# lashhw/rtcuda

Hardware: AMD Instinct MI355X
Metric: Msamples/s at 1920x1080, bun_zipper.ply (higher is better)
Workload: dtype f32

## Files before the change

### rtcuda_amd/csrc/rt_device.h

```cpp
#ifndef RT_DEVICE_H
#define RT_DEVICE_H

#include <hip/hip_runtime.h>
#include <stdint.h>

#include "rt_pinned_math.h"

#define RT_DEV __device__ __forceinline__
#ifdef RT_ISA_MARKS
#define RT_MARK(name) __asm__ volatile("; RT_MARK " name)
#else
#define RT_MARK(name)
#endif

namespace rt {

constexpr float kInvPi = 0.31830988618379067153f;
constexpr float kTwoPi = 6.28318530717958647692f;
constexpr int kRrStart = 4;
constexpr float kRrThreshold = 1.f;
constexpr float kFltMax = 3.402823466e+38f;
constexpr float kFltEps = 1.192092896e-07f;

struct V3 {
    float x, y, z;
};
RT_DEV V3 mk(float x, float y, float z) { return V3{x, y, z}; }
RT_DEV V3 neg(V3 a) { return mk(-a.x, -a.y, -a.z); }
RT_DEV V3 add(V3 a, V3 b) { return mk(a.x + b.x, a.y + b.y, a.z + b.z); }
RT_DEV V3 sub(V3 a, V3 b) { return mk(a.x - b.x, a.y - b.y, a.z - b.z); }
RT_DEV V3 mul(V3 a, V3 b) { return mk(a.x * b.x, a.y * b.y, a.z * b.z); }
RT_DEV V3 scale(V3 a, float t) { return mk(a.x * t, a.y * t, a.z * t); }
RT_DEV V3 divf(V3 a, float t) {
    float inv_t = 1.f / t;
    return mk(a.x * inv_t, a.y * inv_t, a.z * inv_t);
}
RT_DEV float dot(V3 a, V3 b) { return a.x * b.x + a.y * b.y + a.z * b.z; }
RT_DEV V3 cross(V3 a, V3 b) {
    return mk(a.y * b.z - a.z * b.y, a.z * b.x - a.x * b.z, a.x * b.y - a.y * b.x);
}
RT_DEV float len2(V3 a) { return a.x * a.x + a.y * a.y + a.z * a.z; }
RT_DEV float len(V3 a) { return sqrtf(a.x * a.x + a.y * a.y + a.z * a.z); }
RT_DEV V3 unit(V3 a) {
    float inv_len = 1.f / len(a);
    return mk(a.x * inv_len, a.y * inv_len, a.z * inv_len);
}
RT_DEV float max3(V3 a) { return fmaxf(fmaxf(a.x, a.y), a.z); }
template <int STEPS = 1>
RT_DEV float rcp_exact_normal(float x) {
    float r = __builtin_amdgcn_rcpf(x);
#pragma unroll
    for (int k = 0; k < STEPS; k++) {
        const float e = fmaf(-x, r, 1.f);
        r = fmaf(e, r, r);
    }
    return r;
}
RT_DEV V3 reflect(V3 v, V3 n) { return sub(v, scale(n, 2.f * dot(v, n))); }
RT_DEV V3 refract4(V3 unit_v, V3 unit_n, float eta_ratio, float cos_theta) {
    V3 v_parallel = scale(add(unit_v, scale(unit_n, cos_theta)), eta_ratio);
    V3 v_perp = scale(unit_n, -sqrtf(1.f - len2(v_parallel)));
    return add(v_parallel, v_perp);
}

struct Rng {
    uint32_t d, v0, v1, v2, v3, v4;
};
constexpr uint32_t kRngWeyl = 362437u;
RT_DEV void rng_step(Rng &s) {
    uint32_t t = s.v0 ^ (s.v0 >> 2);
    s.v0 = s.v1;
    s.v1 = s.v2;
    s.v2 = s.v3;
    s.v3 = s.v4;
    s.v4 = (s.v4 ^ (s.v4 << 4)) ^ (t ^ (t << 1));
}
RT_DEV uint32_t rng_next(Rng &s) {
    rng_step(s);
    s.d += kRngWeyl;
    return s.v4 + s.d;
}
RT_DEV Rng rng_sample_stream(uint32_t seed_lo, uint32_t seed_hi, unsigned long long key) {
    unsigned long long z = (((unsigned long long)seed_hi << 32) | seed_lo) + 0x9E3779B97F4A7C15ull * (key + 1ull);
    z = (z ^ (z >> 30)) * 0xBF58476D1CE4E5B9ull;
    z = (z ^ (z >> 27)) * 0x94D049BB133111EBull;
    z ^= z >> 31;
    const uint32_t s0 = (uint32_t)z ^ 0xaad26b49u, s1 = (uint32_t)(z >> 32) ^ 0xf7dcefddu;
    const uint32_t t0 = 1099087573u * s0, t1 = 2591861531u * s1;
    Rng r;
    r.d = 6615241u + t1 + t0;
    r.v0 = 123456789u + t0;
    r.v1 = 362436069u ^ t0;
    r.v2 = 521288629u + t1;
    r.v3 = 88675123u ^ t1;
    r.v4 = 5783321u + t0;
    return r;
}
RT_DEV float rng_to_uniform(uint32_t draw) { return (float)draw * 2.3283064e-10f + (2.3283064e-10f / 2.0f); }
RT_DEV float rng_uniform(Rng &s) { return rng_to_uniform(rng_next(s)); }

struct Tri {
    V3 p0, e1, e2, n;
};
RT_DEV Tri load_tri(const float4 *__restrict__ tris, int k) {
    const float4 *q = (const float4 *)((const char *)tris + __umul24((unsigned)k, 48u));
    float4 a = q[0];
    float4 b = q[1];
    float4 c = q[2];
    Tri t;
    t.p0 = mk(a.x, a.y, a.z);
    t.e1 = mk(a.w, b.x, b.y);
    t.e2 = mk(b.z, b.w, c.x);
    t.n = mk(c.y, c.z, c.w);
    return t;
}
RT_DEV bool tri_intersect(const Tri &tr, V3 o, V3 d, float tmax, float &t_out, float &u_out, float &v_out) {
    V3 c = sub(tr.p0, o);
    V3 r = cross(d, c);
    float inv_det = 1.f / dot(d, tr.n);
    float u = inv_det * dot(tr.e2, r);
    float v = inv_det * dot(tr.e1, r);
    float t = inv_det * dot(c, tr.n);
    t_out = t;
    u_out = u;
    v_out = v;
    return u >= 0.0f && v >= 0.0f && (u + v) <= 1.0f && 0 < t && t <= tmax;
}
RT_DEV V3 tri_point(const Tri &tr, float u, float v) { return add(sub(tr.p0, scale(tr.e1, u)), scale(tr.e2, v)); }
RT_DEV float tri_area(const Tri &tr) { return 0.5f * len(tr.n); }

RT_DEV V3 offset_ray_origin(V3 p, V3 n) {
    const float int_scale = 256.f;
    const float float_scale = 1.f / 65536.f;
    const float origin = 1.f / 32.f;
    int ox = (int)(int_scale * n.x);
    int oy = (int)(int_scale * n.y);
    int oz = (int)(int_scale * n.z);
    float px = __int_as_float(__float_as_int(p.x) + (p.x < 0 ? -ox : ox));
    float py = __int_as_float(__float_as_int(p.y) + (p.y < 0 ? -oy : oy));
    float pz = __int_as_float(__float_as_int(p.z) + (p.z < 0 ? -oz : oz));
    return mk(fabsf(p.x) < origin ? p.x + float_scale * n.x : px,
              fabsf(p.y) < origin ? p.y + float_scale * n.y : py,
              fabsf(p.z) < origin ? p.z + float_scale * n.z : pz);
}
RT_DEV float power_heuristic(float f_pdf, float g_pdf_float) {
    int g = (int)g_pdf_float;
    float f2 = f_pdf * f_pdf;
    return f2 / (f2 + (float)(g * g));
}
RT_DEV bool same_hemisphere(V3 wo, V3 wi, V3 n) { return dot(wo, n) * dot(wi, n) < 0.f; }
RT_DEV V3 uniform_sample_sphere(Rng &rs) {
    float z = 1 - 2 * rng_uniform(rs);
    float r = sqrtf(1 - z * z);
    float phi = kTwoPi * rng_uniform(rs);
    float x, y;
    rt_sincosf(phi, &y, &x);
    return mk(r * x, r * y, z);
}

struct Material {
    float ax, ay, az;
    float ior;
    int type;
};
RT_DEV bool mat_get_f(const Material &m, V3 wo, V3 wi, V3 n, V3 &f, float &pdf) {
    if (m.type == 0) {
        if (same_hemisphere(wo, wi, n)) {
            f = scale(mk(m.ax, m.ay, m.az), kInvPi);
            pdf = dot(wi, n) * kInvPi;
            return true;
        }
    }
    return false;
}
RT_DEV V3 mat_sample_f(const Material &m, V3 wo, Rng &rs, V3 &n, V3 &wi, float &pdf, int &again_draws) {
    again_draws = 0;
    if (m.type == 0 || m.type == 1) {
        if (dot(wo, n) > 0.f) n = neg(n);
        if (m.type == 0) {
            again_draws = 2;
            wi = unit(add(n, uniform_sample_sphere(rs)));
            pdf = dot(wi, n) * kInvPi;
            return scale(mk(m.ax, m.ay, m.az), kInvPi);
        } else {
            wi = reflect(wo, n);
            pdf = 1.f;
            return divf(mk(m.ax, m.ay, m.az), dot(wi, n));
        }
    } else {
        float cos_theta = dot(wo, n);
        bool front = cos_theta < 0.f;
        if (front) cos_theta = -cos_theta;
        float inv_cos = 1.f / cos_theta;
        float eta = front ? 1.f / m.ior : m.ior;
        float sin_theta = sqrtf(1.f - cos_theta * cos_theta);
        bool cannot_refract = eta * sin_theta > 1.f;
        if (cannot_refract) {
            if (!front) n = neg(n);
            wi = reflect(wo, n);
            pdf = 1.f;
            return mk(inv_cos, inv_cos, inv_cos);
        }
        again_draws = 1;
        float r0 = (1 - m.ior) / (1 + m.ior);
        r0 = r0 * r0;
        float reflectance = r0 + (1 - r0) * rt_pow5f(1 - cos_theta);
        if (rng_uniform(rs) < reflectance) {
            if (!front) n = neg(n);
            wi = reflect(wo, n);
            pdf = reflectance;
            float v = pdf * inv_cos;
            return mk(v, v, v);
        } else {
            if (!front) n = neg(n);
            wi = refract4(wo, n, eta, cos_theta);
            n = neg(n);
            pdf = 1.f - reflectance;
            float v = pdf * eta * eta / dot(wi, n);
            return mk(v, v, v);
        }
    }
}
struct Light {
    int type;
    float px, py, pz;
    int tri;
    float lx, ly, lz;
};

struct Camera {
    V3 lookfrom, upper_left, horizontal, vertical;
};
RT_DEV void camera_get_ray(const Camera &c, float x, float y, V3 &o, V3 &d) {
    V3 dir = sub(add(add(c.upper_left, scale(c.horizontal, x)), scale(c.vertical, y)), c.lookfrom);
    o = c.lookfrom;
    d = unit(dir);
}

}
#endif
```

### rtcuda_amd/csrc/rt_frame_kernels.inc

```
#ifndef RT_CHUNK_RELEASE_WAIT
#define RT_CHUNK_RELEASE_WAIT 1
#endif

template <class SRC, bool LDS_TABLES>
__global__ void __launch_bounds__(kBlock)
k_advance(DScene sc, DPools p, SRC cam, AdvanceParams ap, float *__restrict__ fb, DCounters *__restrict__ ctr,
             DWaveRow *__restrict__ rows, unsigned int *__restrict__ lock_shades) {
    if (ap.lockstep >= 3 && lock_shades[ap.lockstep - 2] == 0u) return;
    __shared__ float s_tab[LDS_TABLES ? kTabDwordsMax : 1];
    const int i = blockIdx.x * blockDim.x + threadIdx.x;
    const bool in_range = i < ap.n;
    SlotState st;
    st.bounces = kDone;
    st.hit_info = -1;
    st.pixel = 0;
    st.gen = 0;
    st.rs = Rng{0, 0, 0, 0, 0, 0};
    st.beta = st.wo = st.isect_p = st.isect_n = mk(0, 0, 0);
    if (in_range) {
        st.bounces = p.bounces(i);
        st.hit_info = p.hit_info(i);
        st.pixel = p.pixel(i);
        st.gen = p.gen(i);
        st.rs = Rng{p.rd(i), p.r0(i), p.r1(i), p.r2(i), p.r3(i), p.r4(i)};
        st.beta = mk(p.br(i), p.bg(i), p.bb(i));
        st.wo = mk(p.dx(i), p.dy(i), p.dz(i));
        st.isect_p = mk(p.hpx(i), p.hpy(i), p.hpz(i));
        st.isect_n = mk(p.hnx(i), p.hny(i), p.hnz(i));
    }
    const float *tab = sc.tables;
    if (LDS_TABLES) {
        for (int k = threadIdx.x; k < sc.tab_dwords; k += kBlock) s_tab[k] = sc.tables[k];
        __syncthreads();
        tab = s_tab;
    }
    if (ap.lockstep && st.bounces == kParked) {
        st.bounces = ap.max_bounces;
        st.hit_info = -1;
    }
    const bool alive = st.bounces != kDone && st.bounces != kParked;
    AdvanceOut out;
    out.did_gen = out.did_shade = out.has_shadow = out.did_emit = out.new_ray = false;
    out.rr_draws = 0;
    if (alive) {
        const int gen_before = st.gen;
        advance_core<false>(sc, tab, cam, ap, ap.slot_lo + i, st, out, fb);
        if (out.new_ray) {
            p.ox(i) = out.ray_o.x;
            p.oy(i) = out.ray_o.y;
            p.oz(i) = out.ray_o.z;
            p.dx(i) = out.ray_d.x;
            p.dy(i) = out.ray_d.y;
            p.dz(i) = out.ray_d.z;
        }
        if (st.gen != gen_before) {
            p.gen(i) = st.gen;
            p.pixel(i) = st.pixel;
        }
        if (out.has_shadow) {
            p.sox(i) = out.s_o.x;
            p.soy(i) = out.s_o.y;
            p.soz(i) = out.s_o.z;
            p.sdx(i) = out.s_d.x;
            p.sdy(i) = out.s_d.y;
            p.sdz(i) = out.s_d.z;
            p.slr(i) = out.s_L.x;
            p.slg(i) = out.s_L.y;
            p.slb(i) = out.s_L.z;
            p.starget(i) = out.s_target;
            p.stmax(i) = out.s_tmax;
        }
        p.br(i) = st.beta.x;
        p.bg(i) = st.beta.y;
        p.bb(i) = st.beta.z;
        p.bounces(i) = st.bounces;
        p.rd(i) = st.rs.d;
        p.r0(i) = st.rs.v0;
        p.r1(i) = st.rs.v1;
        p.r2(i) = st.rs.v2;
        p.r3(i) = st.rs.v3;
        p.r4(i) = st.rs.v4;
    }
    if (in_range && !out.has_shadow) p.stmax(i) = -1.f;

    unsigned long long traced = wave_ballot(out.did_gen || out.did_shade);
    int rr_tot = out.rr_draws;
    if (wave_ballot(out.rr_draws != 0)) {
        for (int off = 32; off > 0; off >>= 1) rr_tot += __shfl_xor(rr_tot, off);
    } else {
        rr_tot = 0;
    }
    unsigned long long v[C_COUNT] = {(unsigned long long)wave_count((out.did_gen)),
                                     (unsigned long long)wave_count((out.did_shade)),
                                     (unsigned long long)__popcll(traced),
                                     (unsigned long long)wave_count((out.has_shadow)),
                                     (unsigned long long)wave_count((out.did_emit)),
                                     0ull,
                                     (unsigned long long)rr_tot,
                                     0ull};
    row_add(rows, v);
    if ((ap.round & ap.batch_mask) == ap.batch_mask && traced != 0 && lane_id() == 0) ctr->last_live_round = ap.round;
    if (ap.lockstep) {
        unsigned long long sm = wave_ballot(out.did_shade);
        if (sm != 0 && lane_id() == 0) atomicAdd(&lock_shades[ap.lockstep - 1], (unsigned)__popcll(sm));
    }
}

template <class BUILD, bool LDS_TABLES, bool WIDE, int MIN_WAVES, bool DRAW_CIDS = false, bool LITERAL = false, bool VERIFY = false>
__global__ void __launch_bounds__(kBlock, MIN_WAVES)
k_paths(DScene sc, DPools p, typename BUILD::Src cam_arg, AdvanceParams ap_arg, float *__restrict__ fb, DWaveRow *__restrict__ rows,
        int stack_cap, int *overflow, int adv_batch, int debug_no_deposit, unsigned long long *prof, int top_n,
        int prio_period, int rot_wave, int rot_set, int gen_batch, int tri_follow, unsigned int *__restrict__ next_cid,
        unsigned long long *__restrict__ vstat) {
    using SRC = typename BUILD::Src;
    constexpr bool SPLIT_GEN = MIN_WAVES != 2;
    asm volatile("s_nop 0\n\ts_nop 0");
    extern __shared__ int s_lds[];
    int *stack = s_lds + threadIdx.x;
    float *park = (float *)(s_lds + (stack_cap + 1) * kBlock) + threadIdx.x;
    int *over = overflow + (blockIdx.x * kBlock + threadIdx.x) % kOverStride;
    int *cold = s_lds + (stack_cap + 10) * kBlock + threadIdx.x;
    float *acc = (float *)(s_lds + (stack_cap + 23) * kBlock) + threadIdx.x;
    float *s_tab = (float *)(s_lds + (stack_cap + 26) * kBlock);
    const float *tab = sc.tables;
    const float4 *s_top = (const float4 *)(s_tab + (LDS_TABLES ? ((sc.tab_dwords + 3) & ~3) : 0));
    constexpr bool CHUNKS = BUILD::kChunks && SPLIT_GEN && !DRAW_CIDS;
    __shared__ __attribute__((aligned(16))) unsigned s_task[CHUNKS ? 8 : 1];
    __shared__ unsigned s_sem[CHUNKS ? rtchunks::kSemWords : 1];
    const unsigned chunk_g0 = (CHUNKS && top_n > 0) ? (unsigned)top_n & ((1u << rtplan::kChunkHeadShift) - 1u) : 0u;
    const unsigned chunk_head0 = (CHUNKS && top_n > 0) ? (unsigned)top_n >> rtplan::kChunkHeadShift : 0u;
    if (CHUNKS) {
        for (unsigned k = threadIdx.x; k < rtchunks::kSemWords; k += kBlock) s_sem[k] = rtchunks::kSemWordInit;
        if (threadIdx.x == 0) {
            const rtchunks::Multiple m = rtchunks::multiple_of(chunk_g0 ? chunk_g0 : 1u);
            s_task[0] = 0u;
            s_task[1] = chunk_g0;
            s_task[2] = m.inv;
            s_task[3] = m.shift;
            s_task[4] = m.limit;
            s_task[5] = chunk_head0;
            if constexpr (BUILD::kBg) s_task[6] = rtchunks::next_multiple_mul(chunk_g0 ? chunk_g0 : 1u);
        }
    }
    const bool chunk_start = CHUNKS && chunk_g0 && chunk_head0 == 0u;
    if (MIN_WAVES != 2) top_n = 0;
    for (int k = threadIdx.x; k < top_n * 4; k += kBlock) ((float4 *)s_top)[k] = sc.nodes[k];
    if (LDS_TABLES) {
        for (int k = threadIdx.x; k < sc.tab_dwords; k += kBlock) s_tab[k] = sc.tables[k];
        tab = s_tab;
    }
    struct Uniforms {
        SRC cam;
        AdvanceParams ap;
    };
    static_assert(sizeof(Uniforms) % 4 == 0, "dword copy");
    Uniforms *s_uni = (Uniforms *)(s_top + 4 * (size_t)top_n);
    {
        Uniforms u;
        u.cam = cam_arg;
        u.ap = ap_arg;
        const int *srcw = (const int *)&u;
        for (int k = threadIdx.x; k < (int)(sizeof(Uniforms) / 4); k += kBlock) ((int *)s_uni)[k] = srcw[k];
    }
    __syncthreads();
    const SRC &cam = s_uni->cam;
    const AdvanceParams &ap = s_uni->ap;
    const int ap_n = ap_arg.n, ap_max_bounces = ap_arg.max_bounces, ap_fb_fixed = ap_arg.fb_fixed;
    constexpr bool draw_cids = DRAW_CIDS && SPLIT_GEN;
    int cid_next = 0, cid_end = 0;
    int cid_plo = 0, cid_phi = 0;
    unsigned cid_win = 0u;
    const int lanes_in_grid = (int)(gridDim.x * blockDim.x);
    auto slot_of = [&](int set, unsigned lane_in_wg) {
        return rtchunks::slot_of((unsigned)set, blockIdx.x * blockDim.x + lane_in_wg, (unsigned)lanes_in_grid, (unsigned)rot_wave, (unsigned)rot_set);
    };
    int slot_set = 0;
    int i = slot_of(0, threadIdx.x);
    int bounces = kDone, pixel = 0, gen = 0;
    Rng rs{0, 0, 0, 0, 0, 0};
    V3 beta = mk(0, 0, 0);
    auto load_slot = [&](int k) {
        bounces = p.bounces(k);
        pixel = p.pixel(k);
        gen = p.gen(k);
        rs = Rng{p.rd(k), p.r0(k), p.r1(k), p.r2(k), p.r3(k), p.r4(k)};
        beta = mk(p.br(k), p.bg(k), p.bb(k));
    };
    auto store_slot = [&](int k) {
        p.bounces(k) = bounces;
        p.pixel(k) = pixel;
        p.gen(k) = gen;
        p.hit_info(k) = -1;
        p.stmax(k) = -1.f;
        p.br(k) = beta.x;
        p.bg(k) = beta.y;
        p.bb(k) = beta.z;
        p.rd(k) = rs.d;
        p.r0(k) = rs.v0;
        p.r1(k) = rs.v1;
        p.r2(k) = rs.v2;
        p.r3(k) = rs.v3;
        p.r4(k) = rs.v4;
    };
    auto cold_save = [&]() {
        cold[0 * kBlock] = bounces;
        cold[1 * kBlock] = pixel;
        cold[2 * kBlock] = gen;
        cold[3 * kBlock] = (int)rs.d;
        cold[4 * kBlock] = (int)rs.v0;
        cold[5 * kBlock] = (int)rs.v1;
        cold[6 * kBlock] = (int)rs.v2;
        cold[7 * kBlock] = (int)rs.v3;
        cold[8 * kBlock] = (int)rs.v4;
        cold[9 * kBlock] = __float_as_int(beta.x);
        cold[10 * kBlock] = __float_as_int(beta.y);
        cold[11 * kBlock] = __float_as_int(beta.z);
    };
    auto cold_rng = [&]() {
        return Rng{(uint32_t)cold[3 * kBlock], (uint32_t)cold[4 * kBlock], (uint32_t)cold[5 * kBlock],
                   (uint32_t)cold[6 * kBlock], (uint32_t)cold[7 * kBlock], (uint32_t)cold[8 * kBlock]};
    };
    auto cold_load = [&]() {
        bounces = cold[0 * kBlock];
        pixel = cold[1 * kBlock];
        gen = cold[2 * kBlock];
        rs = cold_rng();
        beta = mk(__int_as_float(cold[9 * kBlock]), __int_as_float(cold[10 * kBlock]), __int_as_float(cold[11 * kBlock]));
    };
    auto cold_save_gen = [&](int b, int g, const Rng &r) {
        cold[0 * kBlock] = b;
        cold[2 * kBlock] = g;
        cold[3 * kBlock] = (int)r.d;
        cold[4 * kBlock] = (int)r.v0;
        cold[5 * kBlock] = (int)r.v1;
        cold[6 * kBlock] = (int)r.v2;
        cold[7 * kBlock] = (int)r.v3;
        cold[8 * kBlock] = (int)r.v4;
    };
    int phase = PH_IDLE;
    int tri = -1;
    V3 o = mk(0, 0, 0), d = mk(0, 0, 0), inv = mk(0, 0, 0);
    float tmax = 0.f, hu = 0.f, hv = 0.f;
    int cur = kEntryDone, sp = 0;
    auto next_slot = [&](int first_phase) {
        cold_load();
        store_slot(i);
        phase = PH_IDLE;
        tri = -1;
        slot_set++;
        i = slot_of(slot_set, threadIdx.x);
        if (i < ap_n) {
            load_slot(i);
            if (bounces != kDone && bounces != kParked) {
                phase = first_phase;
                cold_save();
                cold[12 * kBlock] = -1;
            } else {
                i = ap_n;
            }
        }
    };
    int pend = kEntryDone;
    acc[0 * kBlock] = acc[1 * kBlock] = acc[2 * kBlock] = 0.f;
    if (chunk_start) {
        i = ap_n;
        phase = PH_GEN;
        cold[12 * kBlock] = -1;
    } else if (i < ap_n) {
        load_slot(i);
// ... 666 lines not shown
```

### rtcuda_amd/csrc/rtcuda_amd.hip

```cpp
#include <hip/hip_runtime.h>

#include <algorithm>
#include <chrono>
#include <cmath>
#include <cstdio>
#include <cstring>
#include <memory>
#include <mutex>
#include <thread>
#include <type_traits>
#include <string>
#include <vector>

#include "../../include/rtcuda_amd.h"
#include "rt_background.h"
#include "rt_bvh.h"
#include "rt_denoise.h"
#include "rt_device.h"
#include "rt_launch_plan.h"
#include "rt_ploc.h"
#include "rt_ref_tree.h"
#include "rt_slot_chunks.h"
#include "rt_stats_merge.h"
#include "rt_temporal.h"
// ... 341 lines not shown
    while (true) {
        const int step = (hi - lo) / 64 + 1;
        const int probe = min(lo + lane * step, hi);
        const unsigned long long below = wave_ballot(offset[probe] <= c);
        const int j = (int)__popcll(below) - 1;
        const int at = min(lo + j * step, hi);
        if (step == 1) return at;
        hi = min(at + step - 1, hi);
        lo = at;
    }
}
__device__ __forceinline__ void counts_locate(const CountsCamera &s, unsigned c, int lo, int hi, int width, int &pixel, int &px, int &py,
                                              unsigned long long &key) {
    const uint32_t *offset = s.offset;
    const int32_t *first = s.first;
    pixel = counts_find(offset, lo, hi, c);
    const unsigned k = (first ? (unsigned)first[pixel] : 0u) + (c - offset[pixel]);
    key = (unsigned long long)(unsigned)pixel * s.stride + k;
    py = (int)((unsigned)pixel / (unsigned)width);
    px = pixel - py * width;
}
#ifndef RT_RAYS_NONTEMPORAL
#define RT_RAYS_NONTEMPORAL 1
#endif
template <class T>
__device__ __forceinline__ T table_load(const T *q) {
    return RT_RAYS_NONTEMPORAL ? __builtin_nontemporal_load(q) : *q;
}

template <bool NEVER_LOCKSTEP>
__device__ __forceinline__ bool gen_begin(const AdvanceParams &ap, int slot_global, SlotState &st, long long cid_given, long long &cid) {
    const bool lockstep = NEVER_LOCKSTEP ? false : (ap.lockstep != 0);
    cid = cid_given >= 0 ? cid_given : (long long)st.gen * kW + slot_global;
    if (cid >= ap.cam_end) {
        st.bounces = kDone;
        return false;
    }
    if (!lockstep && st.gen == ap.last_gen) {
        st.bounces = kParked;
        return false;
    }
    st.gen = st.gen + 1;
    return true;
}
__device__ __forceinline__ void gen_pixel(const AdvanceParams &ap, int slot_global, SlotState &st, int *pxy, long long cid_given,
                                          long long cid, int &px, int &py) {
    if (cid_given >= 0) {
        st.pixel = (int)((unsigned)cid / (unsigned)ap.spp);
        py = (int)((unsigned)st.pixel / (unsigned)ap.width);
        px = st.pixel - py * ap.width;
    } else if (pxy && ap.dpy >= 0 && *pxy >= 0) {
        px = (*pxy & 0xffff) + ap.dpx;
        py = (*pxy >> 16) + ap.dpy;
        if (px >= ap.width) {
            px -= ap.width;
            py++;
        }
        st.pixel = py * ap.width + px;
    } else {
        if (ap.w_over_spp) st.pixel = (st.gen - 1) * ap.w_over_spp + (int)((unsigned)slot_global / (unsigned)ap.spp);
        else st.pixel = (int)(cid / ap.spp);
        py = (int)((unsigned)st.pixel / (unsigned)ap.width);
        px = st.pixel - py * ap.width;
    }
    if (pxy) *pxy = px | (py << 16);
}
__device__ __forceinline__ bool gen_background(const AdvanceParams &ap, int px, int py) {
    return (unsigned)(px - ap.bg_x0) >= (unsigned)ap.bg_w || (unsigned)(py - ap.bg_y0) >= (unsigned)ap.bg_h;
}
__device__ __forceinline__ void gen_new_path(SlotState &st, AdvanceOut &out) {
    out.new_ray = true;
    st.bounces = 0;
    st.beta = mk(1.f, 1.f, 1.f);
    out.did_gen = true;
}
template <class TABLE>
__device__ __forceinline__ void gen_table_ray(const TABLE &tab, unsigned c, AdvanceOut &out) {
    const float *o3 = tab.o3 + 3 * (size_t)c, *d3 = tab.d3 + 3 * (size_t)c;
    out.ray_o = mk(table_load(o3), table_load(o3 + 1), table_load(o3 + 2));
    out.ray_d = mk(table_load(d3), table_load(d3 + 1), table_load(d3 + 2));
}
__device__ __forceinline__ void gen_camera_ray(const Camera &cam, const AdvanceParams &ap, long long cid, int px, int py, SlotState &st,
                                               AdvanceOut &out) {
    if (ap.per_sample) st.rs = rng_sample_stream(ap.seed_lo, ap.seed_hi, (unsigned long long)cid * (unsigned)ap.key_mul + (unsigned)ap.key_add);
    float jx = rng_uniform(st.rs);
    float jy = rng_uniform(st.rs);
    camera_get_ray(cam, (px + jx) / ap.width, (py + jy) / ap.height, out.ray_o, out.ray_d);
    gen_new_path(st, out);
}

template <bool NEVER_LOCKSTEP = false, bool BG_SKIP = false, class SRC>
__device__ __forceinline__ void gen_core(const SRC &cam, const AdvanceParams &ap, int slot_global, SlotState &st,
                                         AdvanceOut &out, int *pxy = nullptr, long long cid_given = -1) {
    long long cid;
    if constexpr (BG_SKIP && std::is_same<SRC, Camera>::value) {
        int px, py;
        while (true) {
            if (!gen_begin<NEVER_LOCKSTEP>(ap, slot_global, st, cid_given, cid)) return;
            gen_pixel(ap, slot_global, st, pxy, cid_given, cid, px, py);
            if (!gen_background(ap, px, py)) break;
            if (!ap.per_sample) {
                rng_next(st.rs);
                rng_next(st.rs);
            }
            out.bg_skipped++;
        }
        gen_camera_ray(cam, ap, cid, px, py, st, out);
    } else if constexpr (std::is_same<SRC, CountsCamera>::value) {
        int px, py;
        unsigned long long key;
        while (true) {
            if (!gen_begin<NEVER_LOCKSTEP>(ap, slot_global, st, cid_given, cid)) return;
            counts_locate(cam, (unsigned)cid, 0, cam.n_pixels - 1, ap.width, st.pixel, px, py, key);
            if (!BG_SKIP || !gen_background(ap, px, py)) break;
            out.bg_skipped++;
        }
        st.rs = rng_sample_stream(ap.seed_lo, ap.seed_hi, key);
        const float jx = rng_uniform(st.rs);
        const float jy = rng_uniform(st.rs);
        camera_get_ray(cam.cam, (px + jx) / ap.width, (py + jy) / ap.height, out.ray_o, out.ray_d);
        gen_new_path(st, out);
    } else {
        if (!gen_begin<NEVER_LOCKSTEP>(ap, slot_global, st, cid_given, cid)) return;
        if constexpr (std::is_same<SRC, KeyedRayTable>::value) {
            const unsigned c = (unsigned)cid;
            const unsigned long long ck = (unsigned long long)c * cam.key_stride;
            st.rs = rng_sample_stream(ap.seed_lo, ap.seed_hi, cam.key_first + ck);
            rng_next(st.rs);
            rng_next(st.rs);
            gen_table_ray(cam, c, out);
            if (cam.pixel) {
                st.pixel = table_load(cam.pixel + c);
            } else {
                const unsigned long long t = cam.rem_first + ck;
                const unsigned q = (t >> 32) ? (unsigned)(t / cam.rays_per_pixel) : (unsigned)t / cam.rays_per_pixel;
                st.pixel = cam.pix_first + (int)q;
            }
            gen_new_path(st, out);
        } else if constexpr (std::is_same<SRC, RayTable>::value) {
            const unsigned c = (unsigned)cid;
            rng_next(st.rs);
            rng_next(st.rs);
            gen_table_ray(cam, c, out);
            st.pixel = cam.pixel ? table_load(cam.pixel + c) : (int)(c / (unsigned)ap.spp);
            gen_new_path(st, out);
        } else {
            int px, py;
            gen_pixel(ap, slot_global, st, pxy, cid_given, cid, px, py);
            gen_camera_ray(cam, ap, cid, px, py, st, out);
        }
    }
}

template <bool DEFER_GEN, bool NEVER_LOCKSTEP = false, bool USE_ACC = false, bool BG_SKIP = false, class SRC>
__device__ __forceinline__ void advance_core(const DScene &sc, const float *tab, const SRC &cam,
                                             const AdvanceParams &ap, int slot_global, SlotState &st, AdvanceOut &out,
                                             float *__restrict__ fb, float *acc = nullptr) {
    const bool lockstep = NEVER_LOCKSTEP ? false : (ap.lockstep != 0);
    const int off_ltri = tab_off_ltri(sc.num_mats, sc.num_lights);
    const int off_lpre = tab_off_lpre(sc.num_mats, sc.num_lights);
    out.did_gen = out.did_shade = out.has_shadow = out.did_emit = out.new_ray = out.wants_gen = false;
    out.rr_draws = 0;
    out.bg_skipped = 0;
    const bool hit = st.hit_info >= 0;
    const int light_of_hit = hit ? ((st.hit_info >> 16) & 0xffff) - 1 : -1;
    RT_MARK("adv.init");
    if (st.bounces == 0 && hit && light_of_hit >= 0) {
        Light l = tab_light(tab, sc.num_mats, light_of_hit);
        if (USE_ACC) acc_add(acc, l.lx, l.ly, l.lz);
        else deposit(fb, ap.fb_fixed, st.pixel, l.lx, l.ly, l.lz);
        out.did_emit = true;
    }
    const bool cont = st.bounces < ap.max_bounces;
    if (cont && hit) {
        bool shade = true;
        if (st.bounces > kRrStart && max3(st.beta) < kRrThreshold) {
            const float pt = fmaxf(0.05f, 1 - max3(st.beta));
            const int limit = lockstep ? 1 : ap.max_bounces - st.bounces;
            int n = 0;
            uint32_t draw;
            bool kill;
            RT_MARK("adv.rr.begin");
            do {
                n++;
                rng_step(st.rs);
                st.rs.d += kRngWeyl;
                draw = st.rs.v4 + st.rs.d;
                kill = rng_to_uniform(draw) < pt;
            } while (kill & (n < limit));
            RT_MARK("adv.rr.end");
            __asm__ volatile("" : "+v"(draw));
            shade = !(rng_to_uniform(draw) < pt);
            st.bounces = st.bounces + n;
            out.rr_draws = n;
            if (shade) st.beta = divf(st.beta, 1 - pt);
        } else {
            st.bounces = st.bounces + 1;
        }
        if (shade) out.did_shade = true;
        else if (lockstep) return;
    } else {
        if (cont && lockstep) {
            st.bounces = st.bounces + 1;
            return;
        }
    }
    if (!out.did_shade) {
        if (DEFER_GEN) {
            out.wants_gen = true;
            return;
        }
        if (USE_ACC) acc_flush(acc, fb, ap.fb_fixed, st.pixel);
        gen_core<NEVER_LOCKSTEP, BG_SKIP>(cam, ap, slot_global, st, out);
        return;
    }
    RT_MARK("adv.mat.sample_f");
    Material m = tab_material(tab, st.hit_info & 0xffff);
    V3 multiplier = scale(st.beta, (float)sc.num_lights);
    int again_draws;
    {
        V3 n = st.isect_n, wi;
        float pdf;
        V3 f = mat_sample_f(m, st.wo, st.rs, n, wi, pdf, again_draws);
        out.ray_o = offset_ray_origin(st.isect_p, n);
        out.ray_d = wi;
        out.new_ray = true;
        st.beta = mul(st.beta, divf(scale(f, dot(wi, n)), pdf));
    }
    RT_MARK("adv.mat.light_sample");
    if (sc.num_lights > 0) {
        int light_idx = min((int)(rng_uniform(st.rs) * sc.num_lights), sc.num_lights - 1);
        Light light = tab_light(tab, sc.num_mats, light_idx);
        V3 wi, Li;
        float lt, lpdf;
        if (light.type == 0) {
            wi = sub(mk(light.px, light.py, light.pz), st.isect_p);
            lt = len(wi);
            Li = divf(mk(light.lx, light.ly, light.lz), lt * lt);
            wi = divf(wi, lt);
            lpdf = 1.f;
        } else {
            const float *q = tab + off_ltri + 12 * light_idx;
            const float *pre = tab + off_lpre + 4 * light_idx;
            Tri lt_tri;
            lt_tri.p0 = mk(q[0], q[1], q[2]);
            lt_tri.e1 = mk(q[3], q[4], q[5]);
            lt_tri.e2 = mk(q[6], q[7], q[8]);
            lt_tri.n = mk(q[9], q[10], q[11]);
            lpdf = pre[0];
            V3 lun = mk(pre[1], pre[2], pre[3]);
            float a = sqrtf(rng_uniform(st.rs));
            float u2 = rng_uniform(st.rs);
            V3 tp = tri_point(lt_tri, 1 - a, u2 * a);
            wi = sub(tp, st.isect_p);
            lt = len(wi);
            wi = divf(wi, lt);
            Li = mk(light.lx, light.ly, light.lz);
            lpdf *= len2(sub(tp, st.isect_p)) / fabsf(dot(lun, wi));
        }
        RT_MARK("adv.mat.nee");
        V3 n = dot(st.isect_n, wi) > 0.f ? st.isect_n : neg(st.isect_n);
        V3 f;
        float spdf;
        if (mat_get_f(m, st.wo, wi, n, f, spdf)) {
            f = scale(f, dot(wi, n));
            out.s_o = offset_ray_origin(st.isect_p, n);
            out.s_d = wi;
            out.s_tmax = lt;
            out.s_target = light.type == 1 ? light.tri : -1;
            if (light.type == 0) {
                out.s_L = divf(mul(mul(multiplier, f), Li), lpdf);
            } else {
                float weight = power_heuristic(lpdf, spdf);
                out.s_L = divf(scale(mul(mul(multiplier, f), Li), weight), lpdf);
            }
            out.has_shadow = true;
        }
        RT_MARK("adv.mat.burn");
        if (light.type != 0) {
            if (again_draws >= 1) rng_next(st.rs);
            if (again_draws >= 2) rng_next(st.rs);
        }
    }
    RT_MARK("adv.mat.end");
}


#include "rt_walk.inc"
#include "rt_stream_kernels.inc"

enum { PH_ADV = 0, PH_ANY = 1, PH_CLOSEST = 2, PH_IDLE = 3, PH_GEN = 4 };
#ifndef RT_TRI_PER_STEP
#define RT_TRI_PER_STEP 2
#endif
constexpr int kCidChunk = 512;
constexpr int kTriPerStep = RT_TRI_PER_STEP;
#ifndef RT_NODE_PER_STEP
#define RT_NODE_PER_STEP 8
#endif
constexpr int kNodePerStep = RT_NODE_PER_STEP;
#ifndef RT_NODE_PER_STEP_WIDE
#define RT_NODE_PER_STEP_WIDE 2
#endif
constexpr int kNodePerStepWide = RT_NODE_PER_STEP_WIDE;
#ifndef RT_NODE_CONT
#define RT_NODE_CONT 36
#endif
#ifndef RT_NODE_EXTRA
#define RT_NODE_EXTRA 2
#endif
constexpr int kNodeCont = RT_NODE_CONT, kNodeExtra = RT_NODE_EXTRA;
#ifndef RT_SPECULATE
#define RT_SPECULATE 1
#endif

constexpr bool kSpeculate = RT_SPECULATE != 0;

#ifdef RT_TRACE_PROFILE
constexpr int kProfHead = 26;
constexpr int kProfRec = 6;
#endif
struct PathsCamera {
    using Src = Camera;
    static constexpr bool kChunks = false, kBg = false, kCounts = false;
};
struct PathsRays {
    using Src = RayTable;
    static constexpr bool kChunks = false, kBg = false, kCounts = false;
};
struct PathsKeyed {
    using Src = KeyedRayTable;
    static constexpr bool kChunks = false, kBg = false, kCounts = false;
};
struct PathsChunked {
    using Src = Camera;
    static constexpr bool kChunks = true, kBg = false, kCounts = false;
};
struct PathsBg {
    using Src = Camera;
    static constexpr bool kChunks = false, kBg = true, kCounts = false;
};
struct PathsChunkedBg {
    using Src = Camera;
    static constexpr bool kChunks = true, kBg = true, kCounts = false;
};
struct PathsCounts {
    using Src = CountsCamera;
    static constexpr bool kChunks = false, kBg = true, kCounts = true;
};
#include "rt_frame_kernels.inc"

constexpr int kCountsItems = 4, kCountsTile = kCountsItems * 256;
__global__ void __launch_bounds__(256)
k_counts_sums(const int32_t *__restrict__ first, const int32_t *__restrict__ count, int n, uint32_t stride, unsigned long long *__restrict__ words) {
    __shared__ unsigned long long s_sum[4];
    __shared__ unsigned s_bad[4];
    const unsigned base = (blockIdx.x * 256u + threadIdx.x) * (unsigned)kCountsItems;
    unsigned long long sum = 0;
    unsigned bad = 0;
    for (unsigned k = 0; k < (unsigned)kCountsItems; k++) {
        const unsigned p = base + k;
        if (p < (unsigned)n) {
            const long long c = count[p], f = first ? first[p] : 0;
            const bool b = c < 0 || f < 0 || f + c > (long long)stride;
            bad += b ? 1u : 0u;
            sum += b ? 0ull : (unsigned long long)c;
        }
    }
    for (int off = 32; off > 0; off >>= 1) {
        sum += __shfl_xor(sum, off);
        bad += __shfl_xor(bad, off);
    }
    if ((threadIdx.x & 63u) == 0u) {
        s_sum[threadIdx.x >> 6] = sum;
        s_bad[threadIdx.x >> 6] = bad;
    }
    __syncthreads();
    if (threadIdx.x == 0) {
        words[2 + blockIdx.x] = s_sum[0] + s_sum[1] + s_sum[2] + s_sum[3];
        const unsigned b = s_bad[0] + s_bad[1] + s_bad[2] + s_bad[3];
        if (b) atomicAdd(&words[0], (unsigned long long)b);
    }
}
template <class T>
__device__ __forceinline__ T counts_block_scan(T *s, T v) {
    s[threadIdx.x] = v;
    __syncthreads();
    for (unsigned off = 1; off < 256u; off <<= 1) {
        const T t = threadIdx.x >= off ? s[threadIdx.x - off] : (T)0;
        __syncthreads();
        s[threadIdx.x] += t;
        __syncthreads();
    }
    return s[threadIdx.x];
}
__global__ void __launch_bounds__(256) k_counts_scan(unsigned long long *__restrict__ words, int n_tiles) {
    __shared__ unsigned long long s[256];
    unsigned long long carry = 0;
    for (int base = 0; base < n_tiles; base += 256) {
        const int i = base + (int)threadIdx.x;
        const unsigned long long v = i < n_tiles ? words[2 + i] : 0ull;
        const unsigned long long incl = counts_block_scan(s, v);
        const unsigned long long tile_total = s[255];
        if (i < n_tiles) words[2 + i] = carry + incl - v;
        carry += tile_total;
        __syncthreads();
    }
    if (threadIdx.x == 0) words[1] = carry;
}
__global__ void __launch_bounds__(256)
k_counts_offsets(const int32_t *__restrict__ count, int n, const unsigned long long *__restrict__ words, uint32_t *__restrict__ offset,
                 int32_t *__restrict__ samples) {
    __shared__ unsigned s[256];
    const unsigned base = (blockIdx.x * 256u + threadIdx.x) * (unsigned)kCountsItems;
    unsigned c[kCountsItems], mine = 0;
    for (unsigned k = 0; k < (unsigned)kCountsItems; k++) {
        c[k] = base + k < (unsigned)n ? (unsigned)count[base + k] : 0u;
        mine += c[k];
    }
    unsigned at = (unsigned)words[2 + blockIdx.x] + (counts_block_scan(s, mine) - mine);
    for (unsigned k = 0; k < (unsigned)kCountsItems; k++) {
        const unsigned p = base + k;
        if (p < (unsigned)n) {
            offset[p] = at;
            if (samples && c[k]) samples[p] += (int32_t)c[k];
        }
        at += c[k];
    }
    if (blockIdx.x == 0 && threadIdx.x == 0) offset[n] = (unsigned)words[1];
}

__global__ void k_counts_negative(const int32_t *__restrict__ samples, int n, unsigned long long *__restrict__ words) {
    const int i = blockIdx.x * blockDim.x + threadIdx.x;
    const unsigned long long m = wave_ballot(i < n && samples[i] < 0);
    if (m != 0ull && lane_id() == 0) atomicAdd(&words[0], (unsigned long long)__popcll(m));
// ... 514 lines not shown
```

Measured before the change: 5591.

## Precompute xorshift RNG words ahead and select draws instead of branching burn

The shading step now computes the xorshift state words for the next several draws up front and picks them by the BSDF draw count, rather than drawing sequentially and then burning extra draws after light sampling. The final RNG state is rebuilt from the precomputed words with selects, which removes the data-dependent burn branches and serial state shifts. In exchange it computes some words that may go unused and adds register pressure. A prologue s_nop is also trimmed from the frame kernel.

```diff
diff --git a/rtcuda_amd/csrc/rt_device.h b/rtcuda_amd/csrc/rt_device.h
--- a/rtcuda_amd/csrc/rt_device.h
+++ b/rtcuda_amd/csrc/rt_device.h
@@ -67,13 +67,17 @@
     uint32_t d, v0, v1, v2, v3, v4;
 };
 constexpr uint32_t kRngWeyl = 362437u;
+RT_DEV uint32_t rng_word(uint32_t oldest, uint32_t newest) {
+    uint32_t t = oldest ^ (oldest >> 2);
+    return (newest ^ (newest << 4)) ^ (t ^ (t << 1));
+}
 RT_DEV void rng_step(Rng &s) {
-    uint32_t t = s.v0 ^ (s.v0 >> 2);
+    uint32_t w = rng_word(s.v0, s.v4);
     s.v0 = s.v1;
     s.v1 = s.v2;
     s.v2 = s.v3;
     s.v3 = s.v4;
-    s.v4 = (s.v4 ^ (s.v4 << 4)) ^ (t ^ (t << 1));
+    s.v4 = w;
 }
 RT_DEV uint32_t rng_next(Rng &s) {
     rng_step(s);
@@ -98,6 +102,15 @@
 }
 RT_DEV float rng_to_uniform(uint32_t draw) { return (float)draw * 2.3283064e-10f + (2.3283064e-10f / 2.0f); }
 RT_DEV float rng_uniform(Rng &s) { return rng_to_uniform(rng_next(s)); }
+struct Draws {
+    uint32_t w5, w6, d0;
+    int used;
+};
+RT_DEV uint32_t rng_draw(uint32_t word, uint32_t d0, int j) { return word + d0 + (uint32_t)(j + 1) * kRngWeyl; }
+RT_DEV float rng_uniform(Draws &s) {
+    const int j = s.used++;
+    return rng_to_uniform(rng_draw(j == 0 ? s.w5 : s.w6, s.d0, j));
+}
 
 struct Tri {
     V3 p0, e1, e2, n;
@@ -149,7 +162,8 @@
     return f2 / (f2 + (float)(g * g));
 }
 RT_DEV bool same_hemisphere(V3 wo, V3 wi, V3 n) { return dot(wo, n) * dot(wi, n) < 0.f; }
-RT_DEV V3 uniform_sample_sphere(Rng &rs) {
+template <class RS>
+RT_DEV V3 uniform_sample_sphere(RS &rs) {
     float z = 1 - 2 * rng_uniform(rs);
     float r = sqrtf(1 - z * z);
     float phi = kTwoPi * rng_uniform(rs);
@@ -173,7 +187,8 @@
     }
     return false;
 }
-RT_DEV V3 mat_sample_f(const Material &m, V3 wo, Rng &rs, V3 &n, V3 &wi, float &pdf, int &again_draws) {
+template <class RS>
+RT_DEV V3 mat_sample_f(const Material &m, V3 wo, RS &rs, V3 &n, V3 &wi, float &pdf, int &again_draws) {
     again_draws = 0;
     if (m.type == 0 || m.type == 1) {
         if (dot(wo, n) > 0.f) n = neg(n);
diff --git a/rtcuda_amd/csrc/rt_frame_kernels.inc b/rtcuda_amd/csrc/rt_frame_kernels.inc
--- a/rtcuda_amd/csrc/rt_frame_kernels.inc
+++ b/rtcuda_amd/csrc/rt_frame_kernels.inc
@@ -114,7 +114,7 @@
         unsigned long long *__restrict__ vstat) {
     using SRC = typename BUILD::Src;
     constexpr bool SPLIT_GEN = MIN_WAVES != 2;
-    asm volatile("s_nop 0\n\ts_nop 0");
+    asm volatile("s_nop 0");
     extern __shared__ int s_lds[];
     int *stack = s_lds + threadIdx.x;
     float *park = (float *)(s_lds + (stack_cap + 1) * kBlock) + threadIdx.x;
diff --git a/rtcuda_amd/csrc/rtcuda_amd.hip b/rtcuda_amd/csrc/rtcuda_amd.hip
--- a/rtcuda_amd/csrc/rtcuda_amd.hip
+++ b/rtcuda_amd/csrc/rtcuda_amd.hip
@@ -517,6 +517,15 @@
     }
 }
 
+__device__ __forceinline__ uint32_t pick3(int k, uint32_t at0, uint32_t at1, uint32_t at2) { return k == 0 ? at0 : k == 1 ? at1 : at2; }
+__device__ __forceinline__ void rng_resume(Rng &rs, const uint32_t *w, uint32_t d0, int k, int T0, int STRIDE) {
+    rs.d = d0 + __umul24((unsigned)(T0 + k * STRIDE), kRngWeyl);
+    rs.v0 = pick3(k, w[T0 + 0], w[T0 + STRIDE + 0], w[T0 + 2 * STRIDE + 0]);
+    rs.v1 = pick3(k, w[T0 + 1], w[T0 + STRIDE + 1], w[T0 + 2 * STRIDE + 1]);
+    rs.v2 = pick3(k, w[T0 + 2], w[T0 + STRIDE + 2], w[T0 + 2 * STRIDE + 2]);
+    rs.v3 = pick3(k, w[T0 + 3], w[T0 + STRIDE + 3], w[T0 + 2 * STRIDE + 3]);
+    rs.v4 = pick3(k, w[T0 + 4], w[T0 + STRIDE + 4], w[T0 + 2 * STRIDE + 4]);
+}
 template <bool DEFER_GEN, bool NEVER_LOCKSTEP = false, bool USE_ACC = false, bool BG_SKIP = false, class SRC>
 __device__ __forceinline__ void advance_core(const DScene &sc, const float *tab, const SRC &cam,
                                              const AdvanceParams &ap, int slot_global, SlotState &st, AdvanceOut &out,
@@ -582,11 +591,18 @@
     RT_MARK("adv.mat.sample_f");
     Material m = tab_material(tab, st.hit_info & 0xffff);
     V3 multiplier = scale(st.beta, (float)sc.num_lights);
-    int again_draws;
+    RT_MARK("adv.mat.draws");
+    uint32_t w[12] = {st.rs.v0, st.rs.v1, st.rs.v2, st.rs.v3, st.rs.v4};
+    const uint32_t d0 = st.rs.d;
+    w[5] = rng_word(w[0], w[4]);
+    w[6] = rng_word(w[1], w[5]);
+    RT_MARK("adv.mat.bsdf");
+    int k1;
     {
         V3 n = st.isect_n, wi;
         float pdf;
-        V3 f = mat_sample_f(m, st.wo, st.rs, n, wi, pdf, again_draws);
+        Draws u{w[5], w[6], d0, 0};
+        V3 f = mat_sample_f(m, st.wo, u, n, wi, pdf, k1);
         out.ray_o = offset_ray_origin(st.isect_p, n);
         out.ray_d = wi;
         out.new_ray = true;
@@ -594,28 +610,43 @@
     }
     RT_MARK("adv.mat.light_sample");
     if (sc.num_lights > 0) {
-        int light_idx = min((int)(rng_uniform(st.rs) * sc.num_lights), sc.num_lights - 1);
+        RT_MARK("adv.mat.draws");
+        w[7] = rng_word(w[2], w[6]);
+        const uint32_t d_k1 = d0 + __umul24((unsigned)k1, kRngWeyl);
+        RT_MARK("adv.mat.light_pick");
+        int light_idx = min((int)(rng_to_uniform(rng_draw(pick3(k1, w[5], w[6], w[7]), d_k1, 0)) * sc.num_lights), sc.num_lights - 1);
         Light light = tab_light(tab, sc.num_mats, light_idx);
         V3 wi, Li;
         float lt, lpdf;
         if (light.type == 0) {
+            RT_MARK("adv.mat.state");
+            rng_resume(st.rs, w, d0, k1, 1, 1);
+            RT_MARK("adv.mat.point_light");
             wi = sub(mk(light.px, light.py, light.pz), st.isect_p);
             lt = len(wi);
             Li = divf(mk(light.lx, light.ly, light.lz), lt * lt);
             wi = divf(wi, lt);
             lpdf = 1.f;
         } else {
-            const float *q = tab + off_ltri + 12 * light_idx;
+            RT_MARK("adv.mat.draws");
+#pragma unroll
+            for (int j = 8; j < 12; j++) w[j] = rng_word(w[j - 5], w[j - 1]);
+            const uint32_t q_a = rng_draw(pick3(k1, w[6], w[7], w[8]), d_k1, 1);
+            const uint32_t q_u2 = rng_draw(pick3(k1, w[7], w[8], w[9]), d_k1, 2);
+            RT_MARK("adv.mat.state");
+            rng_resume(st.rs, w, d0, k1, 3, 2);
+            RT_MARK("adv.mat.area_light");
+            const float *q_tri = tab + off_ltri + 12 * light_idx;
             const float *pre = tab + off_lpre + 4 * light_idx;
             Tri lt_tri;
-            lt_tri.p0 = mk(q[0], q[1], q[2]);
-            lt_tri.e1 = mk(q[3], q[4], q[5]);
-            lt_tri.e2 = mk(q[6], q[7], q[8]);
-            lt_tri.n = mk(q[9], q[10], q[11]);
+            lt_tri.p0 = mk(q_tri[0], q_tri[1], q_tri[2]);
+            lt_tri.e1 = mk(q_tri[3], q_tri[4], q_tri[5]);
+            lt_tri.e2 = mk(q_tri[6], q_tri[7], q_tri[8]);
+            lt_tri.n = mk(q_tri[9], q_tri[10], q_tri[11]);
             lpdf = pre[0];
             V3 lun = mk(pre[1], pre[2], pre[3]);
-            float a = sqrtf(rng_uniform(st.rs));
-            float u2 = rng_uniform(st.rs);
+            float a = sqrtf(rng_to_uniform(q_a));
+            float u2 = rng_to_uniform(q_u2);
             V3 tp = tri_point(lt_tri, 1 - a, u2 * a);
             wi = sub(tp, st.isect_p);
             lt = len(wi);
@@ -641,11 +672,9 @@
             }
             out.has_shadow = true;
         }
-        RT_MARK("adv.mat.burn");
-        if (light.type != 0) {
-            if (again_draws >= 1) rng_next(st.rs);
-            if (again_draws >= 2) rng_next(st.rs);
-        }
+    } else {
+        RT_MARK("adv.mat.state");
+        rng_resume(st.rs, w, d0, k1, 0, 1);
     }
     RT_MARK("adv.mat.end");
 }
```

New measurement: 5627, median of 6. No clear change (+0.6%).
